# chayanchatterjee/GW-Whisper

Measured on AMD Instinct MI355X. Metric: 1s-strain segments/sec (encoder fwd), higher is better.
Workload: dtype bf16; 1 GPU; whisper-tiny encoder fwd, batch 256 log-mel (80x3000) per GPU, 1500 tokens, random-init weights (BASELINE configs[1]); global_batch=256, parallelism=dp1, encoder=tiny, streams_per_gpu=1

## Files before the change

gw_whisper_amd/csrc/mlp_fused.hip:

```cpp
#include "common.h"

#include <stdlib.h>

#include <type_traits>

namespace gww {

namespace {
constexpr int MF_D = 384;
constexpr int MF_KT = MF_D / 64;
constexpr int MF_OT = MF_D / 32;
constexpr int MF_WAVES = 4, MF_THREADS = 256, MF_BM = 128;
#ifndef GWW_MF_EXP
#define GWW_MF_EXP 0
#endif
#ifndef GWW_MF_ABL
#define GWW_MF_ABL 0
#endif
#ifndef GWW_MF_OLDDMA
#define GWW_MF_OLDDMA 0
#endif
#ifndef GWW_MF_AHEAD
#define GWW_MF_AHEAD 3
#endif
// ... 12 lines not shown
#if GWW_MF_NTLOAD
#define MF_NT " nt"
#else
#define MF_NT ""
#endif
#ifndef GWW_MF_PADNOP
#define GWW_MF_PADNOP 0
#endif
#if GWW_MF_PADNOP
#define MF_PADNOP "s_nop 1\n\t"
#else
#define MF_PADNOP ""
#endif
#ifndef GWW_MF_XLDS
#define GWW_MF_XLDS 0
#endif
#ifndef GWW_MF_XSTNT
#define GWW_MF_XSTNT 0
#endif
#ifndef GWW_MF_XNT
#define GWW_MF_XNT 0
#endif
#if GWW_MF_XNT
#define MF_XNT MF_NT
#else
#define MF_XNT ""
#endif
#ifndef GWW_MF_DMAGAP
#define GWW_MF_DMAGAP 1
#endif
#ifndef GWW_MF_TAIL2
#define GWW_MF_TAIL2 0
#endif
#ifndef GWW_MF_NORM
#define GWW_MF_NORM 1
#endif
#ifndef GWW_MF_XACC
#define GWW_MF_XACC 1
#endif
constexpr int MF_AHEAD = GWW_MF_AHEAD;
constexpr int MF_NST_MAX = MF_AHEAD + 1;
constexpr int MF_TILE = 128 * 64 * 2;
constexpr int MF_GL = 16 / MF_WAVES;
constexpr int MF_FMAX = 1536;
constexpr int MF_SLICE_STRIDE = 144, MF_SLICE_BYTES = 32 * MF_SLICE_STRIDE;
constexpr int MF_OFF_CB = MF_NST_MAX * MF_TILE;
constexpr int MF_OFF_U = MF_OFF_CB + MF_FMAX * 4;
constexpr int MF_OFF_B2 = MF_OFF_U + MF_FMAX * 4;
constexpr int MF_OFF_BO = MF_OFF_B2 + MF_D * 4;
constexpr int MF_OFF_QCB = MF_OFF_BO + MF_D * 4;
constexpr int MF_OFF_SLICE = MF_OFF_QCB + MF_FMAX * 4;
constexpr int MF_LDS = MF_OFF_SLICE + 2 * MF_WAVES * MF_SLICE_BYTES;
static_assert(MF_LDS <= 160 * 1024, "LDS budget");

template <int N>
using MF_FL = std::integral_constant<int, N>;

__device__ __forceinline__ float mf_sum8(float v) {
  v += __builtin_bit_cast(float, __builtin_amdgcn_update_dpp(0, __builtin_bit_cast(int, v), 0xB1, 0xF, 0xF, true));
  v += __builtin_bit_cast(float, __builtin_amdgcn_update_dpp(0, __builtin_bit_cast(int, v), 0x4E, 0xF, 0xF, true));
  v += __builtin_bit_cast(float, __builtin_amdgcn_update_dpp(0, __builtin_bit_cast(int, v), 0x141, 0xF, 0xF, true));
  return v;
}

template <int N>
__device__ __forceinline__ void mf_wait_vmcnt() {
  asm volatile("s_waitcnt vmcnt(%0)" ::"n"(N) : "memory");
}

__device__ __forceinline__ float gelu_sig(float x) {
  const float s = fminf(x * x, 64.0f);
  float q = fmaf(s, 0.0010148164f, -0.1067791331f);
  q = fmaf(s, q, -2.3011178f);
#if GWW_MF_EXP & 32
  const float e = (x * q) * 0.37f;
  return x * ((1.0f + e) * 0.91f);
#else
  const float e = __builtin_amdgcn_exp2f(x * q);
  return x * __builtin_amdgcn_rcpf(1.0f + e);
#endif
}

#ifdef GWW_STAMP
__device__ unsigned long long g_stamp_mlp[24];
#define MSTAMP_DECL unsigned long long _t0 = __builtin_amdgcn_s_memtime(); unsigned long long _acc[20] = {0}; \
  const unsigned long long _tb = _t0, _rb = __builtin_amdgcn_s_memrealtime();
#define MSTAMP(i)                                                  \
  do {                                                             \
    if (GWW_STAMP >= 2 && (i) != 0 && (i) != 3 && (i) != 4 && (i) != 5 && !((i) >= 100)) break; \
    __builtin_amdgcn_sched_barrier(0);                             \
    const unsigned long long _t1 = __builtin_amdgcn_s_memtime();   \
    _acc[(i) >= 100 ? (i) - 100 : (i)] += _t1 - _t0;               \
    _t0 = _t1;                                                     \
    __builtin_amdgcn_sched_barrier(0);                             \
  } while (0)
#define TSTAMP(i) do { if (GWW_STAMP == 3) MSTAMP(100 + (i)); } while (0)
#define MSTAMP_FLUSH                                                                 \
  if (lane == 0) {                                                                   \
    for (int _q = 0; _q < 20; ++_q) atomicAdd(&g_stamp_mlp[_q], _acc[_q]);           \
    atomicAdd(&g_stamp_mlp[21], __builtin_amdgcn_s_memrealtime() - _rb);             \
    atomicAdd(&g_stamp_mlp[22], __builtin_amdgcn_s_memtime() - _tb);                 \
    atomicAdd(&g_stamp_mlp[23], 1ull);                                                \
  }
#else
#define MSTAMP_DECL
#define MSTAMP(i)
#define TSTAMP(i)
#define MSTAMP_FLUSH
#endif
}

__device__ __forceinline__ const float* mf_x0_row(const MfX0& z, const float* X, long g, bool x0, bool& tail, int& seg) {
  tail = false; seg = 0;
  if (!x0) return X + g * MF_D;
  const unsigned b = (unsigned)g / (unsigned)z.T, j = (unsigned)g - b * (unsigned)z.T;
  seg = (int)b;
  tail = (int)j >= z.Tt - 2 && (int)j <= z.T - 2;
  if (tail) return z.pos + (long)j * MF_D;
  return z.xs + ((long)b * z.Tt + ((int)j == z.T - 1 ? z.Tt - 1 : (int)j)) * MF_D;
}

struct MfNoX0 {};
template <int MODE, bool OP, bool X0 = false>
__global__ __launch_bounds__(MF_THREADS, 1) void k_mlp_fused(const float* X, const unsigned short* delta, float* x_out,
                                                            const float* __restrict__ ln_u,
                                                            const float* __restrict__ ln_cb,
                                                            const unsigned short* __restrict__ Wt,
                                                            const float* __restrict__ b2,
                                                            unsigned short* __restrict__ C, long M, int F,
                                                            int stagger_ticks, const float* __restrict__ q_u,
                                                            const float* __restrict__ q_cb,
                                                            unsigned short* __restrict__ q_out, int NQ,
                                                            float* x_next, const float* __restrict__ bo, int keep_x_new,
                                                            const std::conditional_t<X0, MfX0, MfNoX0> z) {
  __shared__ __attribute__((aligned(16))) unsigned char lds[MF_LDS];
  constexpr bool QKV = MODE == 1 || MODE == 2, LNQ = MODE == 2, FIN = MODE == 3;
  static_assert(!X0 || (GWW_MF_NORM && GWW_MF_XACC && (MODE == 2 || (MODE == 1 && OP))), "X0: layer 0's two launches; stages in the u table");
  constexpr bool XACC = GWW_MF_XACC && GWW_MF_NORM && GWW_MF_SCHED && OP && (MODE == 1 || MODE == 3);
  constexpr int MF_NST = MF_AHEAD + 1;
  float* lds_cb = reinterpret_cast<float*>(lds + MF_OFF_CB);
  float* lds_u = reinterpret_cast<float*>(lds + MF_OFF_U);
  float* lds_b2 = reinterpret_cast<float*>(lds + MF_OFF_B2);
  float* lds_bo = reinterpret_cast<float*>(lds + MF_OFF_BO);
  float* lds_qcb = reinterpret_cast<float*>(lds + MF_OFF_QCB);
  constexpr int OP_TILES = OP ? 3 * MF_KT : 0;
  typedef __attribute__((address_space(3))) void* lds_ptr;

  const int tid = threadIdx.x, lane = tid & 63, wave = tid >> 6;
  const int r = lane & 31, hh = lane >> 5;
  const long m_base = (long)blockIdx.x * MF_BM + wave * 32;
  unsigned char* slice = lds + MF_OFF_SLICE + wave * MF_SLICE_BYTES;
  unsigned char* const slice0 = slice;
  const int crow = lane >> 3, cchunk = lane & 7;

  const int wave_u = __builtin_amdgcn_readfirstlane(wave);
  const unsigned lane_off = (unsigned)lane * 16u;
  const unsigned lds_base = (unsigned)(unsigned long long)(lds_ptr)lds;
  auto issue_piece_c = [&](int tile, int stage, auto j_c) {
    constexpr int J = decltype(j_c)::value;
    const unsigned dst = lds_base + (unsigned)(stage * MF_TILE + MF_GL * wave_u * 1024);
    if (GWW_MF_EXP & 8) tile &= 7;
    const unsigned short* src = Wt + ((long)tile * (MF_TILE / 2) + MF_GL * wave_u * 512);
    const unsigned lo = lane_off;
    asm volatile("s_mov_b32 m0, %2\n\ts_nop 0\n\tglobal_load_lds_dwordx4 %0, %1 offset:%3"
                 :
                 : "v"(lo), "s"(src), "s"(dst), "n"(J * 1024)
                 : "memory");
  };
  auto issue_piece = [&](int tile, int stage, int j) {
#if GWW_MF_OLDDMA
    const unsigned dst = lds_base + (unsigned)(stage * MF_TILE + (MF_GL * wave_u + j) * 1024);
    const unsigned short* src = Wt + ((long)tile * (MF_TILE / 2) + (MF_GL * wave_u + j) * 512);
    unsigned keep;
    asm volatile("s_mov_b32 %0, m0\n\ts_mov_b32 m0, %3\n\ts_nop 0\n\tglobal_load_lds_dwordx4 %1, %2\n\ts_mov_b32 m0, %0"
                 : "=&s"(keep) : "v"(lane_off), "s"(src), "s"(dst) : "memory");
#else
    if (j == 0) issue_piece_c(tile, stage, std::integral_constant<int, 0>{});
    else if (j == 1) issue_piece_c(tile, stage, std::integral_constant<int, 1>{});
    else if (j == 2) issue_piece_c(tile, stage, std::integral_constant<int, 2>{});
    else issue_piece_c(tile, stage, std::integral_constant<int, 3>{});
#endif
  };
  auto issue = [&](int tile, int stage) {
#pragma unroll
    for (int j = 0; j < MF_GL; ++j) issue_piece(tile, stage, j);
  };

  MSTAMP_DECL
  auto stage_tables = [&]() {
    for (int i = tid; i < F; i += MF_THREADS) {
      lds_cb[i] = GWW_MF_SCHED ? ln_cb[i] * 0.125f : ln_cb[i];
      if (!GWW_MF_NORM) lds_u[i] = ln_u[i];
    }
    if (!GWW_MF_NORM && FIN) __syncthreads();
    if (!LNQ)
      for (int i = tid; i < MF_D; i += MF_THREADS) lds_b2[i] = XACC ? b2[i] + bo[i] : b2[i];
    if (OP)
      for (int i = tid; i < MF_D; i += MF_THREADS) lds_bo[i] = bo[i];
    if (FIN)
      for (int i = tid; i < MF_D; i += MF_THREADS) { lds_u[i] = q_u[i]; lds_u[MF_D + i] = q_cb[i]; }
    if (QKV && GWW_MF_NORM)
      for (int i = tid; i < NQ; i += MF_THREADS) lds_qcb[i] = q_cb[i];
  };
  if constexpr (!XACC) stage_tables();
  if (stagger_ticks > 0 && blockIdx.x < 256) {
    const unsigned long long t0 = __builtin_amdgcn_s_memrealtime();
    const unsigned long long wait = (unsigned long long)((blockIdx.x >> 3) & 15) * stagger_ticks;
    while (__builtin_amdgcn_s_memrealtime() - t0 < wait) __builtin_amdgcn_s_sleep(8);
  }

#pragma unroll
  for (int p = 0; p < MF_AHEAD; ++p) issue(p, p);
  const long xrow_l = m_base + r < M ? m_base + r : M - 1;
  const unsigned xoff = (unsigned)xrow_l * (unsigned)(MF_D * 4) + 16u * (unsigned)hh;
  f32x4 xp[XACC ? MF_OT : 1][4];
  bool x0 = false;
  int x0_seg0 = 0;
  f32x4* const lds_x0 = reinterpret_cast<f32x4*>(lds + MF_OFF_U);
  const float* x0_stage[2] = {nullptr, nullptr};
  f32x4 x0_sg[2];
  bool x0_tail = false;
  int x0_seg = 0;
  if constexpr (X0) {
    x0 = __builtin_amdgcn_readfirstlane(*z.flag) != 0;
    const unsigned g0 = (unsigned)blockIdx.x * (unsigned)MF_BM;
    x0_seg0 = (int)(g0 / (unsigned)z.T);
    const int seg_last = (int)((unsigned)(M - 1) / (unsigned)z.T);
#pragma unroll
    for (int k = 0; k < 2; ++k) {
      const int q = tid + 256 * k < 4 * (MF_D / 4) ? tid + 256 * k : tid;
      const int sg = q / (2 * (MF_D / 4)), wh = (q / (MF_D / 4)) & 1, c = q % (MF_D / 4);
      const long b = x0_seg0 + sg < seg_last ? x0_seg0 + sg : seg_last;
      x0_stage[k] = (wh ? z.tr + b * MF_D : z.xs + (b * z.Tt + (z.Tt - 2)) * MF_D) + 4 * c;
    }
  }
  auto x0_publish = [&](f32x4 (&sg)[2]) {
    lds_x0[tid] = sg[0];
    if (tid + 256 < 4 * (MF_D / 4)) lds_x0[tid + 256] = sg[1];
    asm volatile("s_waitcnt lgkmcnt(0)" ::: "memory");
    __builtin_amdgcn_s_barrier();
    asm volatile("" ::: "memory");
  };
  if constexpr (XACC && X0) {
    const float* xsrc = mf_x0_row(z, X, xrow_l, x0, x0_tail, x0_seg) + 4 * hh;
#pragma unroll
    for (int t = 0; t < MF_OT; ++t)
#pragma unroll
      for (int cc = 0; cc < 4; ++cc)
        asm volatile("global_load_dwordx4 %0, %1, off offset:%2" MF_XNT : "=a"(xp[t][cc]) : "v"(xsrc), "n"((32 * t + 8 * cc) * 4) : "memory");
#pragma unroll
    for (int k = 0; k < 2; ++k) asm volatile("global_load_dwordx4 %0, %1, off" : "=v"(x0_sg[k]) : "v"(x0_stage[k]) : "memory");
  } else if constexpr (XACC) {
#pragma unroll
    for (int t = 0; t < MF_OT; ++t)
#pragma unroll
      for (int cc = 0; cc < 4; ++cc)
        if (GWW_MF_ABL & 32) asm volatile("v_accvgpr_write_b32 %0, 0" : "=a"(xp[t][cc][0]));
        else asm volatile("global_load_dwordx4 %0, %1, %2 offset:%3" MF_XNT : "=a"(xp[t][cc]) : "v"(xoff), "s"(X), "n"((32 * t + 8 * cc) * 4) : "memory");
  }
  bf16x8 af[MF_KT * 4];
  float row_rstd, row_mean;
  long grow[4];
#pragma unroll
  for (int i = 0; i < 4; ++i) {
    const long g = m_base + 8 * i + crow;
    grow[i] = g < M ? g : M - 1;
  }
  if constexpr (XACC) {
    const unsigned coff = (unsigned)xrow_l * (unsigned)(MF_D * 2) + 64u * (unsigned)hh;
#pragma unroll
    for (int S = 0; S < MF_KT; ++S)
#pragma unroll
      for (int j = 0; j < 4; ++j)
        asm volatile("global_load_dwordx4 %0, %1, %2 offset:%3" : "=v"(af[4 * S + j]) : "v"(coff), "s"(delta), "n"((64 * S + 8 * j) * 2) : "memory");
    if constexpr (X0) {
      if (x0) {
        asm volatile("s_waitcnt vmcnt(24)" : "+v"(x0_sg[0]), "+v"(x0_sg[1]) : : "memory");
#pragma unroll
        for (int t = 0; t < MF_OT; ++t) asm volatile("" : "+a"(xp[t][0]), "+a"(xp[t][1]), "+a"(xp[t][2]), "+a"(xp[t][3]));
        x0_publish(x0_sg);
        if (x0_tail) {
          const f32x4* const st = lds_x0 + (x0_seg - x0_seg0) * (2 * (MF_D / 4)) + hh;
#pragma unroll
          for (int t = 0; t < MF_OT; ++t)
#pragma unroll
            for (int cc = 0; cc < 4; ++cc) {
              const f32x4 xt = st[8 * t + 2 * cc], rt = st[MF_D / 4 + 8 * t + 2 * cc];
#pragma unroll
              for (int k = 0; k < 4; ++k) xp[t][cc][k] = __builtin_fmaf(xt[k], rt[k], xp[t][cc][k]);
            }
        }
      }
    }
    stage_tables();
    asm volatile("s_waitcnt vmcnt(0)" ::: "memory");
#pragma unroll
    for (int i = 0; i < MF_KT * 4; ++i) asm volatile("" : "+v"(af[i]));
    row_rstd = 1.f; row_mean = 0.f;
  } else if constexpr (OP) {
    const unsigned short* crow_p[4];
#pragma unroll
    for (int i = 0; i < 4; ++i) crow_p[i] = delta + grow[i] * MF_D + 8 * cchunk;
    u32x4 cv[MF_KT][4];
#pragma unroll
    for (int S = 0; S < MF_KT; ++S)
#pragma unroll
      for (int i = 0; i < 4; ++i) {
        if (GWW_MF_ABL & 64) { cv[S][i] = u32x4{0x3f803f80u, 0x3f803f80u, 0x3f803f80u, 0x3f803f80u}; continue; }
        asm volatile("global_load_dwordx4 %0, %1, off offset:%2" MF_NT : "=v"(cv[S][i]) : "v"(crow_p[i]), "n"(64 * S * 2) : "memory");
      }
#pragma unroll
    for (int S = 0; S < MF_KT; ++S) {
#pragma unroll
      for (int i = 0; i < 4; ++i) {
        if (!(GWW_MF_ABL & 64)) asm volatile("s_waitcnt vmcnt(%1)" : "+v"(cv[S][i]) : "n"(23 - (4 * S + i)));
        *reinterpret_cast<u32x4*>(slice + (8 * i + crow) * MF_SLICE_STRIDE + cchunk * 16) = cv[S][i];
      }
#pragma unroll
      for (int j = 0; j < 4; ++j) {
        u32x4 u = *reinterpret_cast<const u32x4*>(slice + r * MF_SLICE_STRIDE + (4 * hh + j) * 16);
        asm volatile("" : "+v"(u)::"memory");
        af[4 * S + j] = __builtin_bit_cast(bf16x8, u);
      }
    }
    row_rstd = 1.f; row_mean = 0.f;
  } else
  {
    float s1[4] = {0.f, 0.f, 0.f, 0.f}, s2[4] = {0.f, 0.f, 0.f, 0.f}, cshift[4];
    const float* xrow[4];
    const unsigned short* drow[4];
#pragma unroll
    for (int i = 0; i < 4; ++i) {
      xrow[i] = X + grow[i] * MF_D + 4 * cchunk;
      drow[i] = LNQ ? nullptr : delta + grow[i] * MF_D + 4 * cchunk;
    }
    bool tl[4] = {false, false, false, false};
    const f32x4* st_row[4] = {lds_x0, lds_x0, lds_x0, lds_x0};
    if constexpr (X0) {
#pragma unroll
      for (int i = 0; i < 4; ++i) {
        int seg;
        xrow[i] = mf_x0_row(z, X, grow[i], x0, tl[i], seg) + 4 * cchunk;
        st_row[i] = lds_x0 + (seg - x0_seg0) * (2 * (MF_D / 4)) + cchunk;
      }
#pragma unroll
      for (int k = 0; k < 2; ++k) asm volatile("global_load_dwordx4 %0, %1, off" : "=v"(x0_sg[k]) : "v"(x0_stage[k]) : "memory");
    }
#pragma unroll
    for (int S3 = 0; S3 < MF_KT; S3 += 3) {
      f32x4 xv[3][2][4];
      u32x2 dv[3][2][4];
#pragma unroll
      for (int S = 0; S < 3; ++S)
#pragma unroll
        for (int h2 = 0; h2 < 2; ++h2)
#pragma unroll
          for (int i = 0; i < 4; ++i) {
            if constexpr (X0)
              asm volatile("global_load_dwordx4 %0, %1, off offset:%2"
                           : "=v"(xv[S][h2][i]) : "v"(xrow[i]), "n"((64 * (S3 + S) + 32 * h2) * 4) : "memory");
            else
            asm volatile("global_load_dwordx4 %0, %1, off offset:%2" MF_NT
                         : "=v"(xv[S][h2][i]) : "v"(xrow[i]), "n"((64 * (S3 + S) + 32 * h2) * 4) : "memory");
            if (!LNQ)
              asm volatile("global_load_dwordx2 %0, %1, off offset:%2" MF_NT
                           : "=v"(dv[S][h2][i]) : "v"(drow[i]), "n"((64 * (S3 + S) + 32 * h2) * 2) : "memory");
          }
      if constexpr (X0) {
        if (S3 == 0 && x0) {
          asm volatile("s_waitcnt vmcnt(24)" : "+v"(x0_sg[0]), "+v"(x0_sg[1]) : : "memory");
          x0_publish(x0_sg);
        }
      }
#pragma unroll
      for (int Sl = 0; Sl < 3; ++Sl) {
        const int S = S3 + Sl;
#pragma unroll
// ... 143 lines not shown
    act_val(slot, p, 0); act_val(slot, p, 1); act_val(slot, p, 2); act_val(slot, p, 3);
    act_end(slot, p);
  };

  float g_t[4] = {0.f, 0.f, 0.f, 0.f}, g_w[4] = {0.f, 0.f, 0.f, 0.f}, g_q[4] = {0.f, 0.f, 0.f, 0.f};
#define MF_FENCE()                                                                                                       \
  asm volatile("" : "+v"(g_t[0]), "+v"(g_t[1]), "+v"(g_t[2]), "+v"(g_t[3]), "+v"(g_w[0]), "+v"(g_w[1]), "+v"(g_w[2]),   \
               "+v"(g_w[3]), "+v"(g_q[0]), "+v"(g_q[1]), "+v"(g_q[2]), "+v"(g_q[3]))
  auto preload_bias = [&](int t, int chunk, int q) {
    const float4 bv = *reinterpret_cast<const float4*>(lds_cb + 64 * chunk + 32 * (t & 1) + 8 * q + 4 * hh);
    sacc[t][4 * q] = bv.x; sacc[t][4 * q + 1] = bv.y; sacc[t][4 * q + 2] = bv.z; sacc[t][4 * q + 3] = bv.w;
  };
  auto gelu_slice = [&](int t, int g) {
    if (GWW_MF_EXP & 2) return;
    const int k = g / 12, j = g % 12;
#pragma unroll
    for (int pr = 0; pr < 2; ++pr) {
      const int op = j - pr;
      if (op < 0 || op > 8) continue;
#pragma unroll
      for (int sl = 0; sl < 2; ++sl) {
        const int i = 2 * pr + sl, v = 4 * k + i;
        const float S_ = sacc[t][v];
        float& T_ = g_t[i];
        float& W_ = g_w[i];
        float& Q_ = g_q[i];
        if (op == 0) asm("v_mul_f32_e64 %0, %1, %1 clamp" : "=v"(W_) : "v"(S_));
        else if (op == 1) Q_ = fmaf(W_, 33.2535038f, -54.67091615f);
        else if (op == 2) Q_ = fmaf(W_, Q_, -18.4089424f);
        else if (op == 3) W_ = S_ * Q_;
        else if (op == 4) W_ = __builtin_amdgcn_exp2f(W_);
        else if (op == 5) W_ = 1.0f + W_;
        else if (op == 6) W_ = __builtin_amdgcn_rcpf(W_);
        else if (op == 7) T_ = S_ * W_;
        else if (op == 8 && sl == 1) {
          pf[t][k >> 1][2 * (k & 1) + pr] = pack2bf(g_t[2 * pr], g_t[2 * pr + 1]);
          asm volatile("" : "+v"(pf[t][k >> 1][2 * (k & 1) + pr]));
        }
      }
    }
  };

  TSTAMP(10);
  mf_wait_vmcnt<0>();
  __builtin_amdgcn_s_barrier();
  TSTAMP(11);

  bf16x8 wf[2][4];
  if (!LNQ && !OP) {
#pragma unroll
    for (int t = 0; t < 4; ++t)
      wf[0][t] = *reinterpret_cast<const bf16x8*>(lds + (t & 1) * 8192 + off1[t >> 1]);
  }
  if (OP) {
#pragma unroll
    for (int u = 0; u < 4; ++u) wf[0][u] = *reinterpret_cast<const bf16x8*>(lds + u * 4096 + offq[0]);
  }

  const int nck = F / 64;
  const int total = OP_TILES + 6 * nck + (QKV ? (NQ / 128) * MF_KT : 0);
  int stage = 0;
  int it = 0;

  auto first_off = [&](int kind, int u) -> int {
    return kind == 0 ? (u & 1) * 8192 + off1[u >> 1] : (kind == 1 ? u * 4096 + off2[0] : u * 4096 + offq[0]);
  };

  auto run_tile = [&](auto flat_c, auto kind_c, auto par_c, auto idx3_c, auto ride_t_c, int ride_cpair, int next_kind,
                      auto pre_c, int pre_chunk, auto pad_c) {
    constexpr int KIND = decltype(kind_c)::value, PAR = decltype(par_c)::value, IDX3 = decltype(idx3_c)::value;
    constexpr int RIDE_T = decltype(ride_t_c)::value;
    constexpr bool PAD = decltype(pad_c)::value != 0;
    constexpr bool NOWAIT = decltype(pad_c)::value == 2;
    constexpr int PRE = decltype(pre_c)::value;
    constexpr int ST = (12 % MF_NST == 0) ? ((decltype(flat_c)::value + OP_TILES) % MF_NST) : -1;
    if (ST >= 0) stage = ST;
    if constexpr (!(GWW_MF_EXP & 64)) {
      if (!NOWAIT) mf_wait_vmcnt<MF_GL * (MF_AHEAD - 2)>();
      __builtin_amdgcn_s_barrier();
    }
    MSTAMP(1);
    const int dma_tile = it + MF_AHEAD < total ? it + MF_AHEAD : total - 1;
    const int dma_stage = stage + MF_AHEAD >= MF_NST ? stage + MF_AHEAD - MF_NST : stage + MF_AHEAD;
    const int stage_next = stage + 1 == MF_NST ? 0 : stage + 1;
    MSTAMP(2);
#pragma unroll
    for (int sub = 0; sub < 4; ++sub) {
      bf16x8(&cur)[4] = wf[sub & 1];
      bf16x8(&nxt)[4] = wf[(sub + 1) & 1];
      const unsigned char* Wn = lds + (sub == 3 ? stage_next : stage) * MF_TILE;
      const int j12 = 4 * IDX3 + sub;
      const int v0 = (16 * j12) / 12, v1 = (16 * (j12 + 1)) / 12;
      __builtin_amdgcn_sched_barrier(0);
      constexpr bool DMA_IN_GAPS = GWW_MF_SCHED && GWW_MF_DMAGAP && RIDE_T >= 0;
      if (!(GWW_MF_EXP & 1) && !DMA_IN_GAPS) issue_piece(dma_tile, dma_stage, sub);
      if (!GWW_MF_SCHED && RIDE_T >= 0) {
#pragma unroll
        for (int v = v0; v < v1; ++v) {
          const int p = 4 * RIDE_T + (v >> 2), e = v & 3;
          if (e == 0) act_begin(0, ride_cpair, p);
          act_val(0, p, e);
          if (e == 3) act_end(0, p);
        }
      }
#pragma unroll
      for (int u = 0; u < 4; ++u) {
        if (KIND == 0) {
          const int tl = u & 1;
          const int ks = 2 * sub + (u >> 1);
          const int afi = 4 * (2 * IDX3 + (ks >> 2)) + (ks & 3);
          if (GWW_MF_SCHED && GWW_MF_VACC) {
            if (PAD) asm volatile("s_nop 1\n\tv_mfma_f32_32x32x16_bf16 %0, %1, %2, %0" : "+v"(sacc[2 * PAR + tl]) : "v"(cur[u]), "v"(af[afi]));
            else asm volatile("v_mfma_f32_32x32x16_bf16 %0, %1, %2, %0" : "+v"(sacc[2 * PAR + tl]) : "v"(cur[u]), "v"(af[afi]));
          } else if (IDX3 == 0 && ks == 0) {
            f32x16 z;
#pragma unroll
            for (int j = 0; j < 16; ++j) z[j] = 0.f;
            sacc[2 * PAR + tl] = __builtin_amdgcn_mfma_f32_32x32x16_bf16(cur[u], af[afi], z, 0, 0, 0);
          } else {
            sacc[2 * PAR + tl] = __builtin_amdgcn_mfma_f32_32x32x16_bf16(cur[u], af[afi], sacc[2 * PAR + tl], 0, 0, 0);
          }
        } else {
          if (GWW_MF_SCHED && PAD)
            asm volatile("s_nop 1\n\tv_mfma_f32_32x32x16_bf16 %0, %1, %2, %0"
                         : "+a"(oacc[4 * IDX3 + u]) : "v"(cur[u]), "v"(pf[2 * PAR + (sub >> 1)][sub & 1]));
          else if (GWW_MF_SCHED)
            asm volatile("v_mfma_f32_32x32x16_bf16 %0, %1, %2, %0"
                         : "+a"(oacc[4 * IDX3 + u]) : "v"(cur[u]), "v"(pf[2 * PAR + (sub >> 1)][sub & 1]));
// ... 169 lines not shown
            f32x4* const sp = reinterpret_cast<f32x4*>(reinterpret_cast<char*>(dst) + xoff + (32 * t + 8 * cc) * 4);
            if (GWW_MF_XSTNT) __builtin_nontemporal_store(v, sp);
            else *sp = v;
          }
        }
        if (GWW_MF_XLDS && dst && !(GWW_MF_ABL & 16) && cc == 3) {
#pragma unroll
          for (int i = 0; i < 4; ++i) {
            const f32x4 u = *reinterpret_cast<const f32x4*>(slice0 + (t & 1) * (MF_WAVES * MF_SLICE_BYTES) + (8 * i + crow) * MF_SLICE_STRIDE + cchunk * 16);
            *reinterpret_cast<f32x4*>(reinterpret_cast<char*>(dst) + (unsigned)grow[i] * (unsigned)(MF_D * 4) + 16u * (unsigned)cchunk + t * 128) = u;
          }
        }
        if (t == 0 && cc == 0) {
          const auto sw = __builtin_amdgcn_permlane32_swap(__float_as_uint(v[0]), __float_as_uint(v[0]), false, false);
          csh = hh ? __uint_as_float(sw[0]) : v[0];
        }
        v[0] -= csh; v[1] -= csh; v[2] -= csh; v[3] -= csh;
        s1 += (v[0] + v[1]) + (v[2] + v[3]);
        s2 += (v[0] * v[0] + v[1] * v[1]) + (v[2] * v[2] + v[3] * v[3]);
      }
    {
      const auto a = __builtin_amdgcn_permlane32_swap(__float_as_uint(s1), __float_as_uint(s1), false, false);
      const auto b = __builtin_amdgcn_permlane32_swap(__float_as_uint(s2), __float_as_uint(s2), false, false);
      s1 = __uint_as_float(a[0]) + __uint_as_float(a[1]);
      s2 = __uint_as_float(b[0]) + __uint_as_float(b[1]);
    }
    const float mean_s = s1 * (1.0f / MF_D);
    row_rstd = rsqrtf(fmaxf(s2 * (1.0f / MF_D) - mean_s * mean_s, 0.f) + 1e-5f);
    row_mean = csh + mean_s;
    const float nm = -mean_s * row_rstd;
    asm volatile("" : "+a"(oacc[0]), "+a"(oacc[1]), "+a"(oacc[2]), "+a"(oacc[3]), "+a"(oacc[4]), "+a"(oacc[5]), "+a"(oacc[6]),
                      "+a"(oacc[7]), "+a"(oacc[8]), "+a"(oacc[9]), "+a"(oacc[10]), "+a"(oacc[11]));
#pragma unroll
    for (int S = 0; S < MF_KT; ++S)
#pragma unroll
      for (int cc = 0; cc < 4; ++cc) {
        const float4 be = *reinterpret_cast<const float4*>(sb + 64 * S + 8 * cc + 4 * hh);
        const float4 bo_ = *reinterpret_cast<const float4*>(sb + 64 * S + 32 + 8 * cc + 4 * hh);
        const f32x16& E = oacc[2 * S];
        const f32x16& O = oacc[2 * S + 1];
        const unsigned e0 = pack2bf(fmaf(E[4 * cc] + be.x - csh, row_rstd, nm), fmaf(E[4 * cc + 1] + be.y - csh, row_rstd, nm));
        const unsigned e1 = pack2bf(fmaf(E[4 * cc + 2] + be.z - csh, row_rstd, nm), fmaf(E[4 * cc + 3] + be.w - csh, row_rstd, nm));
        const unsigned o0 = pack2bf(fmaf(O[4 * cc] + bo_.x - csh, row_rstd, nm), fmaf(O[4 * cc + 1] + bo_.y - csh, row_rstd, nm));
        const unsigned o1 = pack2bf(fmaf(O[4 * cc + 2] + bo_.z - csh, row_rstd, nm), fmaf(O[4 * cc + 3] + bo_.w - csh, row_rstd, nm));
        const auto w0 = __builtin_amdgcn_permlane32_swap(e0, o0, false, false);
        const auto w1 = __builtin_amdgcn_permlane32_swap(e1, o1, false, false);
        const u32x4 f = {w0[0], w1[0], w0[1], w1[1]};
        af[4 * S + cc] = __builtin_bit_cast(bf16x8, f);
      }
      }
  };
  if constexpr (OP) {
    static_assert(12 % MF_NST == 0, "OP mode relies on a ring whose depth divides the 12-tile body (4 or 6 stages)");
#pragma unroll
    for (int nt = 0; nt < 3; ++nt) {
#pragma unroll
      for (int kt = 0; kt < MF_KT; ++kt) {
        const int itile = nt * MF_KT + kt;
        if (!(GWW_MF_ABL & 128)) mf_wait_vmcnt<MF_GL * (MF_AHEAD - 2)>();
        __builtin_amdgcn_s_barrier();
        const int st = itile % MF_NST, st_next = (itile + 1) % MF_NST, dma_st = (itile + MF_AHEAD) % MF_NST;
        const int dma_tile = itile + MF_AHEAD < total ? itile + MF_AHEAD : total - 1;
        const bool last = itile == OP_TILES - 1;
#pragma unroll
        for (int sub = 0; sub < 4; ++sub) {
          const int q = 4 * kt + sub;
          bf16x8(&cur)[4] = wf[q & 1];
          bf16x8(&nxt)[4] = wf[(q + 1) & 1];
          const unsigned char* Wn = lds + (sub == 3 ? st_next : st) * MF_TILE;
          if (!(GWW_MF_ABL & 128)) issue_piece(dma_tile, dma_st, sub);
#pragma unroll
          for (int u = 0; u < 4; ++u) {
            asm volatile(MF_PADNOP "v_mfma_f32_32x32x16_bf16 %0, %1, %2, %0" : "+a"(oacc[4 * nt + u]) : "v"(cur[u]), "v"(af[4 * kt + sub]));
            const int off = (last && sub == 3) ? (u & 1) * 8192 + off1[u >> 1] : u * 4096 + offq[(sub + 1) & 3];
            nxt[u] = *reinterpret_cast<const bf16x8*>(Wn + off);
          }
        }
      }
    }
    it = OP_TILES;
    stage = OP_TILES % MF_NST;
    TSTAMP(14);
    asm volatile("s_nop 15\n\ts_nop 15"
                 : "+a"(oacc[0]), "+a"(oacc[1]), "+a"(oacc[2]), "+a"(oacc[3]), "+a"(oacc[4]), "+a"(oacc[5]), "+a"(oacc[6]),
                   "+a"(oacc[7]), "+a"(oacc[8]), "+a"(oacc[9]), "+a"(oacc[10]), "+a"(oacc[11]));
    if constexpr (XACC) {
      seam_x(lds_bo, (keep_x_new && !(GWW_MF_ABL & 256)) ? x_out : nullptr);
    } else {
    seam(X, x_out, lds_bo, [] {});
#if GWW_MF_NORM
    normalise_af();
#endif
#pragma unroll
    for (int t = 0; t < MF_OT; ++t)
#pragma unroll
      for (int j = 0; j < 16; ++j) oacc[t][j] = 0.f;
    }
    TSTAMP(15);
  }
  if constexpr (!LNQ) {
  if (GWW_MF_SCHED) {
#pragma unroll
    for (int t = 0; t < 4; ++t)
#pragma unroll
      for (int q = 0; q < 4; ++q) preload_bias(t, t >> 1, q);
  }
  using IW = std::conditional_t<OP && !XACC && !(GWW_MF_ABL & 32), I2, I1>;
  run_tile(MF_FL<0>{}, I0{}, I0{}, I0{}, IM{}, 0, 0, IM{}, 0, IW{});
  run_tile(MF_FL<1>{}, I0{}, I0{}, I1{}, IM{}, 0, 0, IM{}, 0, IW{});
  run_tile(MF_FL<2>{}, I0{}, I0{}, I2{}, IM{}, 0, 0, IM{}, 0, I1{});
  TSTAMP(12);
  if (GWW_MF_SCHED) asm volatile("s_nop 15\n\ts_nop 15" : "+v"(sacc[0]), "+v"(sacc[1]), "+v"(sacc[2]), "+v"(sacc[3]));
  act_piece(0, 0, 0); act_piece(0, 0, 1); act_piece(0, 0, 2); act_piece(0, 0, 3);
  TSTAMP(13);
  int b = 0;
  for (; b + 2 < nck; b += 2) {
    run_tile(MF_FL<3>{}, I0{}, I1{}, I0{}, I1{}, b >> 1, 0, IM{}, 0, I0{});
    run_tile(MF_FL<4>{}, I0{}, I1{}, I1{}, I1{}, b >> 1, 0, IM{}, 0, I0{});
    run_tile(MF_FL<5>{}, I0{}, I1{}, I2{}, I1{}, b >> 1, 1, IM{}, 0, I0{});
    run_tile(MF_FL<6>{}, I1{}, I0{}, I0{}, I2{}, b >> 1, 1, I0{}, b + 2, I0{});
    run_tile(MF_FL<7>{}, I1{}, I0{}, I1{}, I2{}, b >> 1, 1, IM{}, 0, I0{});
    run_tile(MF_FL<8>{}, I1{}, I0{}, I2{}, I2{}, b >> 1, 0, IM{}, 0, I0{});
    run_tile(MF_FL<9>{}, I0{}, I0{}, I0{}, I3{}, b >> 1, 0, IM{}, 0, I0{});
    run_tile(MF_FL<10>{}, I0{}, I0{}, I1{}, I3{}, b >> 1, 0, IM{}, 0, I0{});
    run_tile(MF_FL<11>{}, I0{}, I0{}, I2{}, I3{}, b >> 1, 1, IM{}, 0, I0{});
    run_tile(MF_FL<12>{}, I1{}, I1{}, I0{}, I0{}, (b >> 1) + 1, 1, I1{}, b + 3, I0{});
    run_tile(MF_FL<13>{}, I1{}, I1{}, I1{}, I0{}, (b >> 1) + 1, 1, IM{}, 0, I0{});
    run_tile(MF_FL<14>{}, I1{}, I1{}, I2{}, I0{}, (b >> 1) + 1, 0, IM{}, 0, I0{});
  }
  run_tile(MF_FL<3>{}, I0{}, I1{}, I0{}, I1{}, b >> 1, 0, IM{}, 0, I1{});
  run_tile(MF_FL<4>{}, I0{}, I1{}, I1{}, I1{}, b >> 1, 0, IM{}, 0, I1{});
  run_tile(MF_FL<5>{}, I0{}, I1{}, I2{}, I1{}, b >> 1, 1, IM{}, 0, I1{});
  run_tile(MF_FL<6>{}, I1{}, I0{}, I0{}, I2{}, b >> 1, 1, IM{}, 0, I1{});
  run_tile(MF_FL<7>{}, I1{}, I0{}, I1{}, I2{}, b >> 1, 1, IM{}, 0, I1{});
// ... 172 lines not shown
    }
  } else {
    if constexpr (XACC) {
      seam_x(lds_b2, x_next);
    } else if constexpr (!LNQ) {
      seam(x_out, x_next, lds_b2, [] {});
#if GWW_MF_NORM
    normalise_af();
#else
      for (int i = tid; i < NQ; i += MF_THREADS) { lds_qcb[i] = q_cb[i]; lds_u[i] = q_u[i]; }
      mf_wait_vmcnt<0>();
#endif
    } else {
      mf_wait_vmcnt<0>();
    }
    __builtin_amdgcn_s_barrier();

    MSTAMP(5);
#if GWW_MF_TAIL2
    {
    const int nchunks = NQ / 64;
    u32x4 tq[4];
#pragma unroll
    for (int i = 0; i < 4; ++i) tq[i] = u32x4{0u, 0u, 0u, 0u};
    auto q_preload = [&](int t, int chunk, int q) {
      const float4 bv = *reinterpret_cast<const float4*>(lds_qcb + 64 * chunk + 32 * (t & 1) + 8 * q + 4 * hh);
      sacc[t][4 * q] = bv.x; sacc[t][4 * q + 1] = bv.y; sacc[t][4 * q + 2] = bv.z; sacc[t][4 * q + 3] = bv.w;
    };
    auto q_ride = [&](auto q_c, auto g_c, int chunk, auto mode_c) {
      constexpr int Q = decltype(q_c)::value, G = decltype(g_c)::value, RM = decltype(mode_c)::value;
      if constexpr (RM == 1 && G >= 4 && G < 12) {
        constexpr int tt = (G - 4) >> 2, cc = (G - 4) & 3;
        const f32x16& a = sacc[2 * Q + tt];
        u32x2 o = {pack2bf(a[4 * cc], a[4 * cc + 1]), pack2bf(a[4 * cc + 2], a[4 * cc + 3])};
        *reinterpret_cast<u32x2*>(slice + r * MF_SLICE_STRIDE + (32 * tt + 8 * cc + 4 * hh) * 2) = o;
      }
      if constexpr (RM >= 1 && G >= 12 && G < 20) {
        if (chunk + 1 < nchunks) q_preload(2 * Q + ((G - 12) >> 2), chunk + 1, (G - 12) & 3);
      }
      if constexpr (RM == 1 && G >= 22 && G < 26) {
        tq[G - 22] = *reinterpret_cast<const u32x4*>(slice + (8 * (G - 22) + crow) * MF_SLICE_STRIDE + cchunk * 16);
        asm volatile("" : "+v"(tq[G - 22]));
      }
      if constexpr (RM == 1 && G >= 37 && G < 41) {
        const long orow = m_base + 8 * (G - 37) + crow;
        if (!(GWW_MF_ABL & 1))
          __builtin_nontemporal_store(tq[G - 37], reinterpret_cast<u32x4*>(q_out + orow * NQ + (chunk - 1) * 64 + 8 * cchunk));
      }
    };
    auto run_qtile = [&](auto flat_c, auto par_c, auto idx3_c, auto mode_c, int chunk, auto extra_c, auto nowait_c) {
      constexpr int FLAT = decltype(flat_c)::value, PAR = decltype(par_c)::value, IDX3 = decltype(idx3_c)::value;
      constexpr int RM = decltype(mode_c)::value, EXTRA = decltype(extra_c)::value;
      constexpr bool NOWAIT = decltype(nowait_c)::value != 0;
      constexpr int ST = (12 % MF_NST == 0) ? ((FLAT + OP_TILES) % MF_NST) : -1;
      if (ST >= 0) stage = ST;
      if (!(GWW_MF_ABL & 4)) {
        if (!NOWAIT) mf_wait_vmcnt<MF_GL*(MF_AHEAD - 2) + ((GWW_MF_ABL & 3) ? 0 : EXTRA)>();
      }
      if (!(GWW_MF_ABL & 8)) __builtin_amdgcn_s_barrier();
      TSTAMP(6);
      const int dma_tile = it + MF_AHEAD < total ? it + MF_AHEAD : total - 1;
      const int dma_stage = stage + MF_AHEAD >= MF_NST ? stage + MF_AHEAD - MF_NST : stage + MF_AHEAD;
      const int stage_next = stage + 1 == MF_NST ? 0 : stage + 1;
#pragma unroll
      for (int sub = 0; sub < 4; ++sub) {
        bf16x8(&cur)[4] = wf[sub & 1];
        bf16x8(&nxt)[4] = wf[(sub + 1) & 1];
        const unsigned char* Wn = lds + (sub == 3 ? stage_next : stage) * MF_TILE;
        __builtin_amdgcn_sched_barrier(0);
#pragma unroll
        for (int u = 0; u < 4; ++u) {
          const int tl = u & 1, ks = 2 * sub + (u >> 1);
          asm volatile("s_nop 1\n\tv_mfma_f32_32x32x16_bf16 %0, %1, %2, %0" : "+v"(sacc[2 * PAR + tl]) : "v"(cur[u]), "v"(af[8 * IDX3 + ks]));
          if (u < 3) asm volatile("" : "+v"(cur[u + 1]));
          else if (sub < 3) asm volatile("" : "+v"(nxt[0]));
          {
            const int off = sub == 3 ? first_off(0, u) : (u & 1) * 8192 + off1[2 * (sub + 1) + (u >> 1)];
            nxt[u] = *reinterpret_cast<const bf16x8*>(Wn + off);
          }
          if constexpr (RM != 0) {
            if (sub == 0 && u == 0) q_ride(MF_FL<1 - PAR>{}, MF_FL<16 * IDX3 + 0>{}, chunk, mode_c);
            else if (sub == 0 && u == 1) q_ride(MF_FL<1 - PAR>{}, MF_FL<16 * IDX3 + 1>{}, chunk, mode_c);
            else if (sub == 0 && u == 2) q_ride(MF_FL<1 - PAR>{}, MF_FL<16 * IDX3 + 2>{}, chunk, mode_c);
            else if (sub == 0 && u == 3) q_ride(MF_FL<1 - PAR>{}, MF_FL<16 * IDX3 + 3>{}, chunk, mode_c);
            else if (sub == 1 && u == 0) q_ride(MF_FL<1 - PAR>{}, MF_FL<16 * IDX3 + 4>{}, chunk, mode_c);
            else if (sub == 1 && u == 1) q_ride(MF_FL<1 - PAR>{}, MF_FL<16 * IDX3 + 5>{}, chunk, mode_c);
            else if (sub == 1 && u == 2) q_ride(MF_FL<1 - PAR>{}, MF_FL<16 * IDX3 + 6>{}, chunk, mode_c);
            else if (sub == 1 && u == 3) q_ride(MF_FL<1 - PAR>{}, MF_FL<16 * IDX3 + 7>{}, chunk, mode_c);
            else if (sub == 2 && u == 0) q_ride(MF_FL<1 - PAR>{}, MF_FL<16 * IDX3 + 8>{}, chunk, mode_c);
            else if (sub == 2 && u == 1) q_ride(MF_FL<1 - PAR>{}, MF_FL<16 * IDX3 + 9>{}, chunk, mode_c);
            else if (sub == 2 && u == 2) q_ride(MF_FL<1 - PAR>{}, MF_FL<16 * IDX3 + 10>{}, chunk, mode_c);
            else if (sub == 2 && u == 3) q_ride(MF_FL<1 - PAR>{}, MF_FL<16 * IDX3 + 11>{}, chunk, mode_c);
            else if (sub == 3 && u == 0) q_ride(MF_FL<1 - PAR>{}, MF_FL<16 * IDX3 + 12>{}, chunk, mode_c);
            else if (sub == 3 && u == 1) q_ride(MF_FL<1 - PAR>{}, MF_FL<16 * IDX3 + 13>{}, chunk, mode_c);
            else if (sub == 3 && u == 2) q_ride(MF_FL<1 - PAR>{}, MF_FL<16 * IDX3 + 14>{}, chunk, mode_c);
            else q_ride(MF_FL<1 - PAR>{}, MF_FL<16 * IDX3 + 15>{}, chunk, mode_c);
          }
          if (!(GWW_MF_ABL & 4)) {
            const int piece = 4 * sub + u - (9 - 4 * IDX3);
            if (piece >= 0 && piece < 4) issue_piece(dma_tile, dma_stage, piece);
          }
        }
        __builtin_amdgcn_sched_barrier(0);
      }
      stage = stage_next;
      ++it;
      TSTAMP(7);
// ... 144 lines not shown
#else
            const float4 bv = *reinterpret_cast<const float4*>(lds_qcb + nl);
            const float4 uv = *reinterpret_cast<const float4*>(lds_u + nl);
            const float v0 = fmaf(row_rstd, fmaf(-row_mean, uv.x, acc[t][4 * cc]), bv.x);
            const float v1 = fmaf(row_rstd, fmaf(-row_mean, uv.y, acc[t][4 * cc + 1]), bv.y);
            const float v2 = fmaf(row_rstd, fmaf(-row_mean, uv.z, acc[t][4 * cc + 2]), bv.z);
            const float v3 = fmaf(row_rstd, fmaf(-row_mean, uv.w, acc[t][4 * cc + 3]), bv.w);
#endif
            u32x2 o = {pack2bf(v0, v1), pack2bf(v2, v3)};
            *reinterpret_cast<u32x2*>(slice + r * MF_SLICE_STRIDE + (32 * tt + 8 * cc + 4 * hh) * 2) = o;
          }
        }
#pragma unroll
        for (int i = 0; i < 4; ++i) {
          const u32x4 u = *reinterpret_cast<const u32x4*>(slice + (8 * i + crow) * MF_SLICE_STRIDE + cchunk * 16);
          const long orow = m_base + 8 * i + crow;
          if (GWW_MF_ABL & 1) { asm volatile("" :: "v"(u)); continue; }
#if GWW_MF_NTSTORE
          __builtin_nontemporal_store(u, reinterpret_cast<u32x4*>(q_out + orow * NQ + nt * 128 + 64 * half + 8 * cchunk));
#else
          *reinterpret_cast<u32x4*>(q_out + orow * NQ + nt * 128 + 64 * half + 8 * cchunk) = u;
#endif
        }
      }
    }
    mf_wait_vmcnt<(GWW_MF_ABL & 3) ? 0 : 8>();
#endif
  }
  MSTAMP(3);
  MSTAMP_FLUSH
}

__device__ __forceinline__ u32x4 mf_scale_bf16x8(u32x4 v, float f) {
#pragma unroll
  for (int j = 0; j < 4; ++j) {
    const float lo = __uint_as_float(v[j] << 16) * f, hi = __uint_as_float(v[j] & 0xffff0000u) * f;
    v[j] = (__float_as_uint(lo) >> 16) | (__float_as_uint(hi) & 0xffff0000u);
  }
  return v;
}

__global__ __launch_bounds__(256) void k_mlp_pack(const unsigned short* __restrict__ w1,
                                                  const unsigned short* __restrict__ w2,
                                                  const unsigned short* __restrict__ wq,
                                                  unsigned short* __restrict__ out, int F, long n_chunks16,
                                                  const unsigned short* __restrict__ wo) {
  const int nck = F / 64, mlp_tiles = 6 * nck, op_tiles = wo ? 3 * MF_KT : 0;
  for (long g = (long)blockIdx.x * 256 + threadIdx.x; g < n_chunks16; g += (long)gridDim.x * 256) {
    const int tile_all = (int)(g >> 10), within = (int)(g & 1023);
    const int row = within >> 3, chunk = (within & 7) ^ ((row >> 1) & 7);
    const int tile = tile_all - op_tiles;
    u32x4 v;
    if (tile < 0) {
      const int nt = tile_all / MF_KT, kt = tile_all - nt * MF_KT;
      v = *reinterpret_cast<const u32x4*>(wo + (long)(128 * nt + row) * MF_D + 64 * kt + 8 * chunk);
    } else if (tile >= mlp_tiles) {
#if GWW_MF_TAIL2
      const int it2 = tile - mlp_tiles, cq = it2 / 3, k3 = it2 - 3 * cq;
      const int row2 = within >> 4, ch = (within & 15) ^ (row2 & 15);
      v = *reinterpret_cast<const u32x4*>(wq + (long)(64 * cq + row2) * MF_D + 128 * k3 + 8 * ch);
#else
      const int it2 = tile - mlp_tiles, nt = it2 / MF_KT, kt = it2 - nt * MF_KT;
      v = *reinterpret_cast<const u32x4*>(wq + (long)(128 * nt + row) * MF_D + 64 * kt + 8 * chunk);
#endif
    } else {
      int kind, cp, idx3;
      if (tile < 3) { kind = 0; cp = 0; idx3 = tile; }
      else {
        const int k = tile - 3, blk = k / 6, w = k - 6 * blk;
        if (blk == nck - 1) { kind = 1; cp = blk; idx3 = w; }
        else if (w < 3) { kind = 0; cp = blk + 1; idx3 = w; }
        else { kind = 1; cp = blk; idx3 = w - 3; }
      }
      if (kind == 0) {
        const int row2 = within >> 4, ch = (within & 15) ^ (row2 & 15);
        v = *reinterpret_cast<const u32x4*>(w1 + (long)(64 * cp + row2) * MF_D + 128 * idx3 + 8 * ch);
        if (GWW_MF_SCHED) v = mf_scale_bf16x8(v, 0.125f);
      } else {
        const unsigned short* src = w2 + (long)(128 * idx3 + row) * F + 64 * cp;
        unsigned short e[8];
#pragma unroll
        for (int j = 0; j < 8; ++j) {
          const int p = 8 * chunk + j;
          e[j] = src[(p & ~12) | ((p & 4) << 1) | ((p & 8) >> 1)];
        }
        v = u32x4{(unsigned)e[0] | ((unsigned)e[1] << 16), (unsigned)e[2] | ((unsigned)e[3] << 16),
                  (unsigned)e[4] | ((unsigned)e[5] << 16), (unsigned)e[6] | ((unsigned)e[7] << 16)};
        if (GWW_MF_SCHED) v = mf_scale_bf16x8(v, 8.0f);
      }
    }
    reinterpret_cast<u32x4*>(out)[g] = v;
  }
}

int launch_mlp_pack(const void* w1_folded, const void* w2, const void* wqkv_folded, void* out, int d, int F, int NQ,
                    hipStream_t s, const void* wo) {
  GWW_REQUIRE(d == MF_D && F % 128 == 0 && F >= 0 && (F > 0 || wqkv_folded),
              "mlp_pack: d must be 384 and ffn a multiple of 128 (0: only the q / k / v panel, for LayerNorm 1 + q / k / v alone)");
  GWW_REQUIRE(!wqkv_folded || (NQ > 0 && NQ % 128 == 0), "mlp_pack: the q / k / v panel needs NQ %% 128 == 0");
  GWW_REQUIRE(!wo || F > 0, "mlp_pack: an out_proj panel goes in front of an MLP stream");
  const long n16 = ((wo ? (long)MF_D * MF_D : 0) + 2L * MF_D * F + (wqkv_folded ? (long)NQ * MF_D : 0)) / 8;
  hipLaunchKernelGGL(k_mlp_pack, dim3((unsigned)cdiv(n16, 256)), dim3(256), 0, s, (const unsigned short*)w1_folded,
                     (const unsigned short*)w2, (const unsigned short*)wqkv_folded, (unsigned short*)out, F, n16,
                     (const unsigned short*)wo);
  GWW_LAUNCH_CHECK();
  return GWW_OK;
}
// ... 154 lines not shown
```

Measured before the change: 25740 segments/s.

## Stream attention-context operand via LDS DMA ring instead of register loads

```diff
diff --git a/gw_whisper_amd/csrc/mlp_fused.hip b/gw_whisper_amd/csrc/mlp_fused.hip
--- a/gw_whisper_amd/csrc/mlp_fused.hip
+++ b/gw_whisper_amd/csrc/mlp_fused.hip
@@ -88,6 +88,10 @@
 constexpr int MF_OFF_SLICE = MF_OFF_QCB + MF_FMAX * 4;
 constexpr int MF_LDS = MF_OFF_SLICE + 2 * MF_WAVES * MF_SLICE_BYTES;
 static_assert(MF_LDS <= 160 * 1024, "LDS budget");
+constexpr int MF_CTX_RING = 2, MF_CTX_PARK = MF_D / 64 - MF_CTX_RING;
+constexpr int MF_LDS_OP = MF_LDS + 2 * MF_TILE;
+constexpr int mf_park_off(int p) { return p < 2 ? MF_OFF_SLICE + p * MF_TILE : MF_LDS + (p - 2) * MF_TILE; }
+static_assert(2 * MF_TILE <= 2 * MF_WAVES * MF_SLICE_BYTES && MF_LDS_OP <= 160 * 1024, "LDS budget (OP)");
 
 template <int N>
 using MF_FL = std::integral_constant<int, N>;
@@ -169,7 +173,7 @@
                                                             unsigned short* __restrict__ q_out, int NQ,
                                                             float* x_next, const float* __restrict__ bo, int keep_x_new,
                                                             const std::conditional_t<X0, MfX0, MfNoX0> z) {
-  __shared__ __attribute__((aligned(16))) unsigned char lds[MF_LDS];
+  __shared__ __attribute__((aligned(16))) unsigned char lds[OP ? MF_LDS_OP : MF_LDS];
   constexpr bool QKV = MODE == 1 || MODE == 2, LNQ = MODE == 2, FIN = MODE == 3;
   static_assert(!X0 || (GWW_MF_NORM && GWW_MF_XACC && (MODE == 2 || (MODE == 1 && OP))), "X0: layer 0's two launches; stages in the u table");
   constexpr bool XACC = GWW_MF_XACC && GWW_MF_NORM && GWW_MF_SCHED && OP && (MODE == 1 || MODE == 3);
@@ -180,6 +184,7 @@
   float* lds_bo = reinterpret_cast<float*>(lds + MF_OFF_BO);
   float* lds_qcb = reinterpret_cast<float*>(lds + MF_OFF_QCB);
   constexpr int OP_TILES = OP ? 3 * MF_KT : 0;
+  constexpr int OP_RING = OP ? OP_TILES + MF_CTX_RING : 0;
   typedef __attribute__((address_space(3))) void* lds_ptr;
 
   const int tid = threadIdx.x, lane = tid & 63, wave = tid >> 6;
@@ -221,6 +226,26 @@
 #pragma unroll
     for (int j = 0; j < MF_GL; ++j) issue_piece(tile, stage, j);
   };
+  unsigned ctx_off[OP ? MF_GL : 1];
+  if constexpr (OP) {
+#pragma unroll
+    for (int j = 0; j < MF_GL; ++j) {
+      const int R = 8 * (MF_GL * wave + j) + (lane >> 3);
+      const long g = (long)blockIdx.x * MF_BM + R;
+      ctx_off[j] = (unsigned)(g < M ? g : M - 1) * (unsigned)(MF_D * 2) + 16u * (unsigned)((lane & 7) ^ ((R >> 1) & 7));
+    }
+  }
+  auto issue_ctx_piece = [&](int kt, int tile_off, int j) {
+    if (GWW_MF_ABL & 64) return;
+    const unsigned dst = lds_base + (unsigned)(tile_off + (MF_GL * wave_u + j) * 1024);
+    const unsigned short* src = delta + 64 * kt;
+    const unsigned vo = ctx_off[j];
+    asm volatile("s_mov_b32 m0, %2\n\ts_nop 0\n\tglobal_load_lds_dwordx4 %0, %1" : : "v"(vo), "s"(src), "s"(dst) : "memory");
+  };
+  auto issue_ring_piece = [&](int ri, int stage, int j, int n_tiles) {
+    if (ri < MF_CTX_RING) issue_ctx_piece(ri, stage * MF_TILE, j);
+    else issue_piece(ri - MF_CTX_RING < n_tiles ? ri - MF_CTX_RING : n_tiles - 1, stage, j);
+  };
 
   MSTAMP_DECL
   auto stage_tables = [&]() {
@@ -245,8 +270,19 @@
     while (__builtin_amdgcn_s_memrealtime() - t0 < wait) __builtin_amdgcn_s_sleep(8);
   }
 
+  if constexpr (OP) {
+#pragma unroll
+    for (int p = 0; p < MF_AHEAD; ++p)
+#pragma unroll
+      for (int j = 0; j < MF_GL; ++j) issue_ring_piece(p, p, j, OP_TILES);
+#pragma unroll
+    for (int p = 0; p < MF_CTX_PARK; ++p)
+#pragma unroll
+      for (int j = 0; j < MF_GL; ++j) issue_ctx_piece(MF_CTX_RING + p, mf_park_off(p), j);
+  } else {
 #pragma unroll
   for (int p = 0; p < MF_AHEAD; ++p) issue(p, p);
+  }
   const long xrow_l = m_base + r < M ? m_base + r : M - 1;
   const unsigned xoff = (unsigned)xrow_l * (unsigned)(MF_D * 4) + 16u * (unsigned)hh;
   f32x4 xp[XACC ? MF_OT : 1][4];
@@ -303,15 +339,9 @@
     grow[i] = g < M ? g : M - 1;
   }
   if constexpr (XACC) {
-    const unsigned coff = (unsigned)xrow_l * (unsigned)(MF_D * 2) + 64u * (unsigned)hh;
-#pragma unroll
-    for (int S = 0; S < MF_KT; ++S)
-#pragma unroll
-      for (int j = 0; j < 4; ++j)
-        asm volatile("global_load_dwordx4 %0, %1, %2 offset:%3" : "=v"(af[4 * S + j]) : "v"(coff), "s"(delta), "n"((64 * S + 8 * j) * 2) : "memory");
     if constexpr (X0) {
       if (x0) {
-        asm volatile("s_waitcnt vmcnt(24)" : "+v"(x0_sg[0]), "+v"(x0_sg[1]) : : "memory");
+        asm volatile("s_waitcnt vmcnt(0)" : "+v"(x0_sg[0]), "+v"(x0_sg[1]) : : "memory");
 #pragma unroll
         for (int t = 0; t < MF_OT; ++t) asm volatile("" : "+a"(xp[t][0]), "+a"(xp[t][1]), "+a"(xp[t][2]), "+a"(xp[t][3]));
         x0_publish(x0_sg);
@@ -330,35 +360,8 @@
     }
     stage_tables();
     asm volatile("s_waitcnt vmcnt(0)" ::: "memory");
-#pragma unroll
-    for (int i = 0; i < MF_KT * 4; ++i) asm volatile("" : "+v"(af[i]));
     row_rstd = 1.f; row_mean = 0.f;
   } else if constexpr (OP) {
-    const unsigned short* crow_p[4];
-#pragma unroll
-    for (int i = 0; i < 4; ++i) crow_p[i] = delta + grow[i] * MF_D + 8 * cchunk;
-    u32x4 cv[MF_KT][4];
-#pragma unroll
-    for (int S = 0; S < MF_KT; ++S)
-#pragma unroll
-      for (int i = 0; i < 4; ++i) {
-        if (GWW_MF_ABL & 64) { cv[S][i] = u32x4{0x3f803f80u, 0x3f803f80u, 0x3f803f80u, 0x3f803f80u}; continue; }
-        asm volatile("global_load_dwordx4 %0, %1, off offset:%2" MF_NT : "=v"(cv[S][i]) : "v"(crow_p[i]), "n"(64 * S * 2) : "memory");
-      }
-#pragma unroll
-    for (int S = 0; S < MF_KT; ++S) {
-#pragma unroll
-      for (int i = 0; i < 4; ++i) {
-        if (!(GWW_MF_ABL & 64)) asm volatile("s_waitcnt vmcnt(%1)" : "+v"(cv[S][i]) : "n"(23 - (4 * S + i)));
-        *reinterpret_cast<u32x4*>(slice + (8 * i + crow) * MF_SLICE_STRIDE + cchunk * 16) = cv[S][i];
-      }
-#pragma unroll
-      for (int j = 0; j < 4; ++j) {
-        u32x4 u = *reinterpret_cast<const u32x4*>(slice + r * MF_SLICE_STRIDE + (4 * hh + j) * 16);
-        asm volatile("" : "+v"(u)::"memory");
-        af[4 * S + j] = __builtin_bit_cast(bf16x8, u);
-      }
-    }
     row_rstd = 1.f; row_mean = 0.f;
   } else
   {
@@ -608,10 +611,6 @@
     for (int t = 0; t < 4; ++t)
       wf[0][t] = *reinterpret_cast<const bf16x8*>(lds + (t & 1) * 8192 + off1[t >> 1]);
   }
-  if (OP) {
-#pragma unroll
-    for (int u = 0; u < 4; ++u) wf[0][u] = *reinterpret_cast<const bf16x8*>(lds + u * 4096 + offq[0]);
-  }
 
   const int nck = F / 64;
   const int total = OP_TILES + 6 * nck + (QKV ? (NQ / 128) * MF_KT : 0);
@@ -629,7 +628,7 @@
     constexpr bool PAD = decltype(pad_c)::value != 0;
     constexpr bool NOWAIT = decltype(pad_c)::value == 2;
     constexpr int PRE = decltype(pre_c)::value;
-    constexpr int ST = (12 % MF_NST == 0) ? ((decltype(flat_c)::value + OP_TILES) % MF_NST) : -1;
+    constexpr int ST = (12 % MF_NST == 0) ? ((decltype(flat_c)::value + OP_RING) % MF_NST) : -1;
     if (ST >= 0) stage = ST;
     if constexpr (!(GWW_MF_EXP & 64)) {
       if (!NOWAIT) mf_wait_vmcnt<MF_GL * (MF_AHEAD - 2)>();
@@ -905,26 +904,53 @@
   };
   if constexpr (OP) {
     static_assert(12 % MF_NST == 0, "OP mode relies on a ring whose depth divides the 12-tile body (4 or 6 stages)");
-#pragma unroll
-    for (int nt = 0; nt < 3; ++nt) {
-#pragma unroll
-      for (int kt = 0; kt < MF_KT; ++kt) {
-        const int itile = nt * MF_KT + kt;
+    bf16x8 cf[2][4];
+    asm volatile("s_nop 1"
+                 : "+a"(oacc[0]), "+a"(oacc[1]), "+a"(oacc[2]), "+a"(oacc[3]), "+a"(oacc[4]), "+a"(oacc[5]), "+a"(oacc[6]),
+                   "+a"(oacc[7]), "+a"(oacc[8]), "+a"(oacc[9]), "+a"(oacc[10]), "+a"(oacc[11]));
+    {
+#pragma unroll
+      for (int c = 0; c < MF_CTX_RING; ++c)
+#pragma unroll
+        for (int j = 0; j < 4; ++j) cf[c][j] = *reinterpret_cast<const bf16x8*>(lds + c * MF_TILE + wave_u * 4096 + offq[j]);
+#pragma unroll
+      for (int u = 0; u < 4; ++u) wf[0][u] = *reinterpret_cast<const bf16x8*>(lds + (MF_CTX_RING % MF_NST) * MF_TILE + u * 4096 + offq[0]);
+      if (!(GWW_MF_ABL & 128)) {
+#pragma unroll
+        for (int j = 0; j < MF_GL; ++j) issue_ring_piece(MF_AHEAD, MF_AHEAD % MF_NST, j, total);
+      }
+      asm volatile("s_waitcnt lgkmcnt(0)" : "+v"(cf[0][0]), "+v"(cf[0][1]), "+v"(cf[0][2]), "+v"(cf[0][3]), "+v"(cf[1][0]), "+v"(cf[1][1]),
+                   "+v"(cf[1][2]), "+v"(cf[1][3]) : : "memory");
+      __builtin_amdgcn_s_barrier();
+      if (!(GWW_MF_ABL & 128)) {
+#pragma unroll
+        for (int j = 0; j < MF_GL; ++j) issue_ring_piece(1 + MF_AHEAD, (1 + MF_AHEAD) % MF_NST, j, total);
+      }
+    }
+#pragma unroll
+    for (int kt = 0; kt < MF_KT; ++kt) {
+#pragma unroll
+      for (int nt = 0; nt < 3; ++nt) {
+        const int ri = MF_CTX_RING + 3 * kt + nt;
         if (!(GWW_MF_ABL & 128)) mf_wait_vmcnt<MF_GL * (MF_AHEAD - 2)>();
         __builtin_amdgcn_s_barrier();
-        const int st = itile % MF_NST, st_next = (itile + 1) % MF_NST, dma_st = (itile + MF_AHEAD) % MF_NST;
-        const int dma_tile = itile + MF_AHEAD < total ? itile + MF_AHEAD : total - 1;
-        const bool last = itile == OP_TILES - 1;
+        const int st = ri % MF_NST, st_next = (ri + 1) % MF_NST, dma_st = (ri + MF_AHEAD) % MF_NST;
+        const bool last = ri == OP_RING - 1;
+        if (nt == 2 && kt + 1 >= MF_CTX_RING && kt + 1 < MF_KT) {
+#pragma unroll
+          for (int j = 0; j < 4; ++j)
+            cf[(kt + 1) & 1][j] = *reinterpret_cast<const bf16x8*>(lds + mf_park_off(kt + 1 - MF_CTX_RING) + wave_u * 4096 + offq[j]);
+        }
 #pragma unroll
         for (int sub = 0; sub < 4; ++sub) {
-          const int q = 4 * kt + sub;
+          const int q = 4 * (3 * kt + nt) + sub;
           bf16x8(&cur)[4] = wf[q & 1];
           bf16x8(&nxt)[4] = wf[(q + 1) & 1];
           const unsigned char* Wn = lds + (sub == 3 ? st_next : st) * MF_TILE;
-          if (!(GWW_MF_ABL & 128)) issue_piece(dma_tile, dma_st, sub);
+          if (!(GWW_MF_ABL & 128)) issue_ring_piece(ri + MF_AHEAD, dma_st, sub, total);
 #pragma unroll
           for (int u = 0; u < 4; ++u) {
-            asm volatile(MF_PADNOP "v_mfma_f32_32x32x16_bf16 %0, %1, %2, %0" : "+a"(oacc[4 * nt + u]) : "v"(cur[u]), "v"(af[4 * kt + sub]));
+            asm volatile(MF_PADNOP "v_mfma_f32_32x32x16_bf16 %0, %1, %2, %0" : "+a"(oacc[4 * nt + u]) : "v"(cur[u]), "v"(cf[kt & 1][sub]));
             const int off = (last && sub == 3) ? (u & 1) * 8192 + off1[u >> 1] : u * 4096 + offq[(sub + 1) & 3];
             nxt[u] = *reinterpret_cast<const bf16x8*>(Wn + off);
           }
@@ -932,7 +958,7 @@
       }
     }
     it = OP_TILES;
-    stage = OP_TILES % MF_NST;
+    stage = OP_RING % MF_NST;
     TSTAMP(14);
     asm volatile("s_nop 15\n\ts_nop 15"
                  : "+a"(oacc[0]), "+a"(oacc[1]), "+a"(oacc[2]), "+a"(oacc[3]), "+a"(oacc[4]), "+a"(oacc[5]), "+a"(oacc[6]),
@@ -1211,7 +1237,7 @@
       constexpr int FLAT = decltype(flat_c)::value, PAR = decltype(par_c)::value, IDX3 = decltype(idx3_c)::value;
       constexpr int RM = decltype(mode_c)::value, EXTRA = decltype(extra_c)::value;
       constexpr bool NOWAIT = decltype(nowait_c)::value != 0;
-      constexpr int ST = (12 % MF_NST == 0) ? ((FLAT + OP_TILES) % MF_NST) : -1;
+      constexpr int ST = (12 % MF_NST == 0) ? ((FLAT + OP_RING) % MF_NST) : -1;
       if (ST >= 0) stage = ST;
       if (!(GWW_MF_ABL & 4)) {
         if (!NOWAIT) mf_wait_vmcnt<MF_GL*(MF_AHEAD - 2) + ((GWW_MF_ABL & 3) ? 0 : EXTRA)>();
@@ -1462,7 +1488,7 @@
     const int tile = tile_all - op_tiles;
     u32x4 v;
     if (tile < 0) {
-      const int nt = tile_all / MF_KT, kt = tile_all - nt * MF_KT;
+      const int kt = tile_all / 3, nt = tile_all - 3 * kt;
       v = *reinterpret_cast<const u32x4*>(wo + (long)(128 * nt + row) * MF_D + 64 * kt + 8 * chunk);
     } else if (tile >= mlp_tiles) {
 #if GWW_MF_TAIL2
```

Result: no change. 25770 segments/s, median of 2 (+0.1%).
